# GradientSpaces/LivingScenes

Measured on AMD Instinct MI355X. Metric: object-instances/sec (encode+match+register), N=1024 pts, higher is better.
Workload: dtype f32 (GEMM products as two-piece f16 splits on the f16 matrix cores, fp32 accumulate: as accurate against fp64 as an fp32 FMA chain)

## Files before the change

### livingscenes_amd/csrc/edge.hip

```cpp
#include "ls_launch.h"
#include "ls_device.h"

namespace ls {

constexpr int EK = 16;

__global__ __launch_bounds__(256) void edge_l0_kernel(const float* __restrict__ pts, const int32_t* __restrict__ knn,
                                                      const float* __restrict__ w0, int N, int Co, float oms,
                                                      float* __restrict__ out, int total) {
    const int lane = threadIdx.x & 63, wave = threadIdx.x >> 6;
    const int sub = lane >> 5, o = lane & 31;
    int pid = (xcd_remap(blockIdx.x, gridDim.x) * 4 + wave) * 2 + sub;
    const bool live = pid < total;
    if (!live) pid = total - 1;
    const int b = pid / N;
    const float* P = pts + (size_t)b * N * 3;
    const float cx = pts[(size_t)pid * 3 + 0], cy = pts[(size_t)pid * 3 + 1], cz = pts[(size_t)pid * 3 + 2];
    const float inv = 1.0f / fmaxf(sqrtf(cx * cx + cy * cy + cz * cz), 1e-12f);
    const float ax = cx * inv, ay = cy * inv, az = cz * inv;
    const int32_t* ki = knn + (size_t)pid * EK;
    __shared__ __attribute__((aligned(16))) float l_edge[4][2][EK][8];
    if (o < EK) {
        const int r = ki[o];
        const float nx = P[(size_t)r * 3 + 0], ny = P[(size_t)r * 3 + 1], nz = P[(size_t)r * 3 + 2];
// ... 250 lines not shown
    for (int col = tid; col < 3 * Co; col += 256) {
        const int ax = col / Co, c = col - ax * Co;
        const float* sp = &l_score[ax * 4 + (c & 3)][c >> 2];
        float a = 0.f;
#pragma unroll
        for (int pw = 0; pw < PW; ++pw) a += sp[(pw / PPW) * 64 + (pw % PPW) * LPP];
        cp[col] = a;
    }
}

template <int LPP, int NCH>
__global__ __launch_bounds__(256) void edge_attn_v4_kernel(const float* __restrict__ T, int ldt, const float* __restrict__ Tq, int ldq,
                                                           int NQ, int q_via_rows, const int32_t* __restrict__ knn,
                                                           const int32_t* __restrict__ dst_rows, int Nd, int Ns, int Co,
                                                           float oms, float inv_sqrt_dk, float* __restrict__ out, int total,
                                                           float* __restrict__ rowmax, float* __restrict__ colsum) {
    constexpr int PPW = 64 / LPP;
    __shared__ float l_score[NCH][EK][256];
    __shared__ float l_ssk[EK][256];
    const int tid = threadIdx.x, lane = tid & 63, wave = tid >> 6;
    const int sub = lane / LPP, ll = lane % LPP;
    int pid = (xcd_remap(blockIdx.x, gridDim.x) * 4 + wave) * PPW + sub;
    const bool live = pid < total;
    if (!live) pid = total - 1;
    const int b = pid / Nd;
    const int drow = (dst_rows && q_via_rows) ? dst_rows[pid] : (pid % Nd);
    const float* Tb = T + (size_t)b * Ns * 3 * ldt;
    const float* Td = Tq + ((size_t)b * NQ + drow) * 3 * ldq;
    const int32_t* ki = knn + (size_t)pid * EK;

    F43 qf[NCH];
    float ssq = 0.f;
#pragma unroll
    for (int ch = 0; ch < NCH; ++ch) {
        const int c4 = (ch * LPP + ll) * 4;
        qf[ch] = ld43(Td + 4 * Co + c4, ldq);
        const F43 kd = ld43(Td + 5 * Co + c4, ldq);
        act43(qf[ch], kd, oms);
        ssq += dot43(qf[ch], qf[ch]);
    }
    const float inv_q = inv_fro(group_sum<LPP>(ssq));

#pragma unroll
    for (int ch = 0; ch < NCH; ++ch) {
        const int c4 = (ch * LPP + ll) * 4;
        const F43 ql = ld43(Td + 2 * Co + c4, ldq), qd = ld43(Td + 3 * Co + c4, ldq);
#pragma unroll 2
        for (int k = 0; k < EK; ++k) {
            const float* Tr = Tb + (size_t)ki[k] * 3 * ldt;
            F43 y = add43(ld43(Tr + 2 * Co + c4, ldt), ql);
            const F43 kd = add43(ld43(Tr + 3 * Co + c4, ldt), qd);
            act43(y, kd, oms);
            const float s2 = dot43(y, y);
            l_ssk[k][tid] = (ch == 0) ? s2 : l_ssk[k][tid] + s2;
            l_score[ch][k][tid] = quad_sum(dot43(y, qf[ch]));
        }
    }
    float mx[NCH], sum[NCH];
#pragma unroll
    for (int ch = 0; ch < NCH; ++ch) { mx[ch] = -INFINITY; sum[ch] = 0.f; }
#pragma unroll 4
    for (int k = 0; k < EK; ++k) {
        const float invk = inv_fro(group_sum<LPP>(l_ssk[k][tid]));
#pragma unroll
        for (int ch = 0; ch < NCH; ++ch) {
            const float v = l_score[ch][k][tid] * inv_q * invk * inv_sqrt_dk;
            l_score[ch][k][tid] = v;
            mx[ch] = fmaxf(mx[ch], v);
        }
    }
#pragma unroll
    for (int ch = 0; ch < NCH; ++ch) {
#pragma unroll 4
        for (int k = 0; k < EK; ++k) {
            const float ex = expf(l_score[ch][k][tid] - mx[ch]);
            l_score[ch][k][tid] = ex;
            sum[ch] += ex;
        }
    }

    float rmx = 0.f, rmy = 0.f, rmz = 0.f;
#pragma unroll
    for (int ch = 0; ch < NCH; ++ch) {
        const int c4 = (ch * LPP + ll) * 4;
        const F43 ql = ld43(Td + c4, ldq), qd = ld43(Td + Co + c4, ldq);
        F43 acc;
        acc.x = acc.y = acc.z = make_float4(0.f, 0.f, 0.f, 0.f);
#pragma unroll 2
        for (int k = 0; k < EK; ++k) {
            const float* Tr = Tb + (size_t)ki[k] * 3 * ldt;
            F43 y = add43(ld43(Tr + c4, ldt), ql);
            const F43 kd = add43(ld43(Tr + Co + c4, ldt), qd);
            act43(y, kd, oms);
            const float w = l_score[ch][k][tid];
            fma43(acc, w, y);
        }
        const float inv = 1.0f / sum[ch];
        const float4 ox = make_float4(acc.x.x * inv, acc.x.y * inv, acc.x.z * inv, acc.x.w * inv);
        const float4 oy = make_float4(acc.y.x * inv, acc.y.y * inv, acc.y.z * inv, acc.y.w * inv);
        const float4 oz = make_float4(acc.z.x * inv, acc.z.y * inv, acc.z.z * inv, acc.z.w * inv);
        if (live) {
            float* op = out + (size_t)pid * 3 * Co + c4;
            *reinterpret_cast<float4*>(op) = ox;
            *reinterpret_cast<float4*>(op + Co) = oy;
            *reinterpret_cast<float4*>(op + 2 * Co) = oz;
        }
        rmx = fmaxf(rmx, amax_f4(ox)); rmy = fmaxf(rmy, amax_f4(oy)); rmz = fmaxf(rmz, amax_f4(oz));
        if constexpr (NCH == 1) {
            if (colsum) attn_colsum<LPP>(l_score[0], ox, oy, oz, live, tid, colsum + (size_t)xcd_remap(blockIdx.x, gridDim.x) * 3 * Co);
        }
    }
    if (rowmax) {
        rmx = group_max<LPP>(rmx); rmy = group_max<LPP>(rmy); rmz = group_max<LPP>(rmz);
        if (live && ll == 0) { float* rp = rowmax + (size_t)pid * 3; rp[0] = rmx; rp[1] = rmy; rp[2] = rmz; }
    }
}


__global__ __launch_bounds__(64) void edge_presplit_wq_kernel(const float* __restrict__ W, int rows, int Cin, int KS, uint4* __restrict__ planes,
                                                               float* __restrict__ winv) {
    const int tile = blockIdx.x / KS, ks = blockIdx.x % KS, lane = threadIdx.x;
    const int n = tile * 32 + (lane & 31), k = ks * 16 + 8 * (lane >> 5);
    const float* wr = W + (size_t)min(n, rows - 1) * Cin;
    float am = 0.f;
    for (int c = 0; c < Cin; ++c) am = fmaxf(am, fabsf(wr[c]));
    float sc, inv;
    pow2_scale(am, sc, inv);
    if (ks == 0 && lane < 32 && n < rows) winv[n] = inv;
    __attribute__((aligned(16))) float v[8];
#pragma unroll
    for (int c = 0; c < 8; ++c) v[c] = wr[k + c] * sc;
    f16x8_t h, l;
    split8_f16(v, h, l);
    planes[((size_t)blockIdx.x * 2) * 64 + lane] = __builtin_bit_cast(uint4, h);
    planes[((size_t)blockIdx.x * 2 + 1) * 64 + lane] = __builtin_bit_cast(uint4, l);
}
static size_t edge_wq_plane_count(int Co, int Cin) { return (size_t)(6 * Co / 32) * (Cin / 16) * 2 * 64; }
size_t edge_wq_planes_bytes(int Co, int Cin) { return edge_wq_plane_count(Co, Cin) * sizeof(uint4) + (size_t)6 * Co * sizeof(float); }
int edge_presplit_wq_launch(const float* Wq, int Co, int Cin, void* planes, hipStream_t st) {
    hipLaunchKernelGGL(edge_presplit_wq_kernel, dim3((6 * Co / 32) * (Cin / 16)), dim3(64), 0, st, Wq, 6 * Co, Cin, Cin / 16, (uint4*)planes,
                       (float*)((uint4*)planes + edge_wq_plane_count(Co, Cin)));
    LS_LAUNCH_CHECK();
    return LS_OK;
}

template <int LPP, int CIN>
__global__ __launch_bounds__(256) __attribute__((amdgpu_waves_per_eu(3))) void edge_attn_fq_kernel(const float* __restrict__ T, int ldt, const float* __restrict__ cur,
                                                           const uint4* __restrict__ Wp, const int32_t* __restrict__ knn,
                                                           const int32_t* __restrict__ dst_rows, int Nd, int Ns, float oms, float inv_sqrt_dk,
                                                           float* __restrict__ out, int total, float* __restrict__ rowmax, float* __restrict__ colsum) {
    constexpr int PPW = 64 / LPP, PW = 4 * PPW, ROWS = 3 * PW, MT = (ROWS + 31) / 32, Co = LPP * 4, SC = 2 * Co, NT = SC / 32, SLD = SC + 4,
                  KS = CIN / 16, ASTR = CIN * 2 + 16;
    static_assert(MT * NT == 8, "two output tiles per wave");
    __shared__ float l_score[EK][256];
    __shared__ __attribute__((aligned(16))) float slab[ROWS * SLD];
    __shared__ __attribute__((aligned(16))) char a_pl[2][MT * 32 * ASTR];
    __shared__ int a_inv[MT * 32];
    const float* __restrict__ winv = reinterpret_cast<const float*>(Wp + (size_t)(6 * Co / 32) * KS * 128);
    const int tid = threadIdx.x, lane = tid & 63, wave = tid >> 6;
    const int sub = lane / LPP, ll = lane % LPP;
    const int pid0 = xcd_remap(blockIdx.x, gridDim.x) * PW;
    const int pwl = wave * PPW + sub;
    int pid = pid0 + pwl;
    const bool live = pid < total;
    if (!live) pid = total - 1;
    const int b = pid / Nd;
    const float* Tb = T + (size_t)b * Ns * 3 * ldt;
    const int32_t* ki = knn + (size_t)pid * EK;
    const int c4 = ll * 4;

    uint4 wfh[2][KS], wfl[2][KS];
    auto qload = [&](int cb) {
        const uint4* wt = Wp + (size_t)(cb / 32) * KS * 128 + lane;
#pragma unroll
        for (int u = 0; u < (MT == 2 ? 1 : 2); ++u) {
            const int nt = MT == 2 ? wave : wave + 4 * u;
#pragma unroll
            for (int ks = 0; ks < KS; ++ks) {
                wfh[u][ks] = wt[((size_t)(nt * KS + ks) * 2) * 64];
                wfl[u][ks] = wt[((size_t)(nt * KS + ks) * 2 + 1) * 64];
            }
        }
    };
    qload(4 * Co);
    for (int c = tid; c < MT * 32 * (CIN / 4); c += 256) {
        const int r = c / (CIN / 4), kq = c - r * (CIN / 4);
        uint2 h = make_uint2(0u, 0u), l = make_uint2(0u, 0u);
        float4 v = make_float4(0.f, 0.f, 0.f, 0.f);
        if (r < ROWS) {
            const int pw = r / 3, x = r - 3 * pw;
            const int pa = min(pid0 + pw, total - 1), ba = pa / Nd;
            const int sp = dst_rows ? dst_rows[pa] : pa - ba * Nd;
            v = *reinterpret_cast<const float4*>(cur + (((size_t)ba * Ns + sp) * 3 + x) * CIN + kq * 4);
        }
        {
            float am = fmaxf(fmaxf(fabsf(v.x), fabsf(v.y)), fmaxf(fabsf(v.z), fabsf(v.w)));
            am = max8(am);
            if constexpr (CIN == 64) am = dpp_max<0x140>(am);
            float sc, inv;
            pow2_scale(am, sc, inv);
            if (kq == 0) a_inv[r] = pow2_e(inv);
            split2_f16_pair(f32x2_t{v.x * sc, v.y * sc}, h.x, l.x);
            split2_f16_pair(f32x2_t{v.z * sc, v.w * sc}, h.y, l.y);
        }
        *reinterpret_cast<uint2*>(&a_pl[0][r * ASTR + kq * 8]) = h;
        *reinterpret_cast<uint2*>(&a_pl[1][r * ASTR + kq * 8]) = l;
    }
    __syncthreads();

    auto qmma = [&](int cb) {
        __builtin_amdgcn_sched_barrier(0);
#pragma unroll
        for (int u = 0; u < 2; ++u) {
            const int mt = MT == 2 ? u : 0, nt = MT == 2 ? wave : wave + 4 * u;
            const int aoff = (32 * mt + (lane & 31)) * ASTR + (lane >> 5) * 16;
            f32x16_t acc;
#pragma unroll
            for (int r = 0; r < 16; ++r) acc[r] = 0.f;
#pragma unroll
            for (int ks = 0; ks < KS; ++ks) {
                const f16x8_t ah = __builtin_bit_cast(f16x8_t, *reinterpret_cast<const uint4*>(&a_pl[0][aoff + ks * 32]));
                const f16x8_t al = __builtin_bit_cast(f16x8_t, *reinterpret_cast<const uint4*>(&a_pl[1][aoff + ks * 32]));
                const f16x8_t bh = __builtin_bit_cast(f16x8_t, wfh[MT == 2 ? 0 : u][ks]);
                const f16x8_t bl = __builtin_bit_cast(f16x8_t, wfl[MT == 2 ? 0 : u][ks]);
                acc = __builtin_amdgcn_mfma_f32_32x32x16_f16(al, bh, acc, 0, 0, 0);
                acc = __builtin_amdgcn_mfma_f32_32x32x16_f16(ah, bh, acc, 0, 0, 0);
                acc = __builtin_amdgcn_mfma_f32_32x32x16_f16(ah, bl, acc, 0, 0, 0);
            }
            const int row0 = 32 * mt + 4 * (lane >> 5);
            float* sp = slab + row0 * SLD + 32 * nt + (lane & 31);
            const int ce = pow2_e(winv[cb + 32 * nt + (lane & 31)]);
#pragma unroll
            for (int r = 0; r < 16; ++r) {
                const int dr = (r & 3) + 8 * (r >> 2);
                if (row0 + dr < ROWS) sp[dr * SLD] = scale_pow2(acc[r], a_inv[row0 + dr] + ce);
            }
        }
    };
    const float* srow = slab + 3 * pwl * SLD + c4;
    auto lds43 = [&](int col) {
        F43 r;
        r.x = *reinterpret_cast<const float4*>(srow + col);
        r.y = *reinterpret_cast<const float4*>(srow + SLD + col);
        r.z = *reinterpret_cast<const float4*>(srow + 2 * SLD + col);
        return r;
    };

    qmma(4 * Co);
    __syncthreads();
    qload(2 * Co);
    F43 qf = lds43(0);
    {
        const F43 kd = lds43(Co);
        act43(qf, kd, oms);
    }
    const float inv_q = inv_fro(group_sum<LPP>(dot43(qf, qf)));
    __syncthreads();

    unsigned nb[EK / 2];
    {
        const int4* kp = reinterpret_cast<const int4*>(ki);
#pragma unroll
        for (int u = 0; u < EK / 4; ++u) { const int4 v = kp[u]; nb[2 * u] = (unsigned)v.x | ((unsigned)v.y << 16); nb[2 * u + 1] = (unsigned)v.z | ((unsigned)v.w << 16); }
    }
    const unsigned row_bytes = 3u * (unsigned)ldt * 4u;
    const unsigned lane_off = (unsigned)c4 * 4u;
    const unsigned inst_row = (unsigned)b * (unsigned)Ns;
    auto noff = [&](int k) { return __umul24(inst_row + ((k & 1) ? nb[k >> 1] >> 16 : nb[k >> 1] & 0xFFFFu), row_bytes) + lane_off; };
    auto ldrow = [&](unsigned off, int col) {
        asm volatile("" : "+v"(off));
        F43 r;
        r.x = *reinterpret_cast<const float4*>(reinterpret_cast<const char*>(T + col) + off);
        r.y = *reinterpret_cast<const float4*>(reinterpret_cast<const char*>(T + ldt + col) + off);
        r.z = *reinterpret_cast<const float4*>(reinterpret_cast<const char*>(T + 2 * ldt + col) + off);
        return r;
    };
    qmma(2 * Co);
    __syncthreads();
    {
        constexpr int DP = 2;
        F43 py[DP], pd[DP];
#pragma unroll
        for (int d = 0; d < DP; ++d) { const unsigned o = noff(d); py[d] = ldrow(o, 2 * Co); pd[d] = ldrow(o, 3 * Co); }
        const F43 ql = lds43(0), qd = lds43(Co);
#pragma unroll
        for (int k = 0; k < EK; ++k) {
            F43 y = py[k % DP], kd = pd[k % DP];
            if (k + DP < EK) { const unsigned o = noff(k + DP); py[k % DP] = ldrow(o, 2 * Co); pd[k % DP] = ldrow(o, 3 * Co); }
            __builtin_amdgcn_sched_barrier(0);
            y = add43(y, ql);
            kd = add43(kd, qd);
            act43(y, kd, oms);
            const float invk = inv_fro(group_sum<LPP>(dot43(y, y)));
            l_score[k][tid] = quad_sum(dot43(y, qf)) * inv_q * invk * inv_sqrt_dk;
            __builtin_amdgcn_sched_barrier(0);
        }
    }
#pragma unroll
    for (int k = 0; k < EK / 2; ++k) asm volatile("" : "+v"(nb[k]));
    __syncthreads();
    qload(0);
    float mx = -INFINITY, sum = 0.f;
#pragma unroll 4
    for (int k = 0; k < EK; ++k) mx = fmaxf(mx, l_score[k][tid]);
#pragma unroll 4
    for (int k = 0; k < EK; ++k) {
        const float ex = expf(l_score[k][tid] - mx);
        l_score[k][tid] = ex;
        sum += ex;
    }
    qmma(0);
    __syncthreads();

    {
        const F43 ql = lds43(0), qd = lds43(Co);
        F43 acc;
        acc.x = acc.y = acc.z = make_float4(0.f, 0.f, 0.f, 0.f);
        constexpr int DP = 2;
        F43 py[DP], pd[DP];
#pragma unroll
        for (int d = 0; d < DP; ++d) { const unsigned o = noff(d); py[d] = ldrow(o, 0); pd[d] = ldrow(o, Co); }
#pragma unroll
        for (int k = 0; k < EK; ++k) {
            F43 y = py[k % DP], kd = pd[k % DP];
            if (k + DP < EK) { const unsigned o = noff(k + DP); py[k % DP] = ldrow(o, 0); pd[k % DP] = ldrow(o, Co); }
            __builtin_amdgcn_sched_barrier(0);
            y = add43(y, ql);
            kd = add43(kd, qd);
            act43(y, kd, oms);
            const float w = l_score[k][tid];
            fma43(acc, w, y);
            __builtin_amdgcn_sched_barrier(0);
        }
        const float inv = 1.0f / sum;
        const float4 ox = make_float4(acc.x.x * inv, acc.x.y * inv, acc.x.z * inv, acc.x.w * inv);
        const float4 oy = make_float4(acc.y.x * inv, acc.y.y * inv, acc.y.z * inv, acc.y.w * inv);
        const float4 oz = make_float4(acc.z.x * inv, acc.z.y * inv, acc.z.z * inv, acc.z.w * inv);
        if (live) {
            float* op = out + (size_t)pid * 3 * Co + c4;
            *reinterpret_cast<float4*>(op) = ox;
            *reinterpret_cast<float4*>(op + Co) = oy;
            *reinterpret_cast<float4*>(op + 2 * Co) = oz;
        }
        if (rowmax) {
            const float rmx = group_max<LPP>(amax_f4(ox)), rmy = group_max<LPP>(amax_f4(oy)), rmz = group_max<LPP>(amax_f4(oz));
            if (live && ll == 0) { float* rp = rowmax + (size_t)pid * 3; rp[0] = rmx; rp[1] = rmy; rp[2] = rmz; }
        }
        if (colsum) attn_colsum<LPP>(l_score, ox, oy, oz, live, tid, colsum + (size_t)(pid0 / PW) * 3 * Co);
    }
}

int edge_l0_launch(const float* pts, const int32_t* knn, const float* w0, int B, int N, int Co, float neg_slope, float* out,
                   hipStream_t st) {
    const int total = B * N;
    hipLaunchKernelGGL(edge_l0_kernel, dim3(cdiv(total, 8)), dim3(256), 0, st, pts, knn, w0, N, Co, 1.0f - neg_slope, out, total);
    LS_LAUNCH_CHECK();
    return LS_OK;
}

int edge_run(const Edge& e, const EdgePlan& p, hipStream_t st) {
    if (p.kernel == EdgeKernel::FT_128 || p.kernel == EdgeKernel::FT_256) return edge_ft_attn_launch(e, p, st);
    const float *T = e.T, *Tq = e.T + p.q_off;
    const int total = e.B * e.Nd, Nd = e.Nd, Ns = e.Ns, Co = e.Co;
    const float oms = 1.0f - e.neg_slope, isd = 1.0f / sqrtf(3.0f * e.head_c);
    float* rowmax = p.rowmax_parts ? e.rowmax : nullptr;
    float* colsum = p.cs_rows ? e.colsum : nullptr;
    const dim3 grid(p.grid), block(p.block);
    LS_REQUIRE(p.kernel < EdgeKernel::ATTN || (e.head_c == 16 && Co % 16 == 0 && p.lds <= 64 * 1024),
               "edge_attn: head width must be 16 and divide Co, Co at most 512 (head_c=%d Co=%d)", e.head_c, Co);
#define LS_POOL(K) hipLaunchKernelGGL(K, grid, block, 0, st, T, p.ldp, Tq, p.ldq, p.NQ, p.qvr, e.knn, e.dst_rows, Nd, Ns, oms, e.out, total)
#define LS_V4(LPP, NCH) hipLaunchKernelGGL((edge_attn_v4_kernel<LPP, NCH>), grid, block, 0, st, T, p.ldp, Tq, p.ldq, p.NQ, p.qvr, e.knn, e.dst_rows, Nd, Ns, Co, oms, isd, e.out, total, rowmax, colsum)
#define LS_FQ(LPP, CIN) hipLaunchKernelGGL((edge_attn_fq_kernel<LPP, CIN>), grid, block, 0, st, T, p.ldp, e.cur, (const uint4*)e.planes, e.knn, e.dst_rows, Nd, Ns, oms, isd, e.out, total, rowmax, colsum)
    switch (p.kernel) {
    case EdgeKernel::ATTN_FQ_16_32: LS_FQ(16, 32); break;
    case EdgeKernel::ATTN_FQ_16_64: LS_FQ(16, 64); break;
    case EdgeKernel::ATTN_FQ_32_64: LS_FQ(32, 64); break;
    case EdgeKernel::POOL_V4_8: LS_POOL(edge_pool_v4_kernel<8>); break;
    case EdgeKernel::POOL_V4_16: LS_POOL(edge_pool_v4_kernel<16>); break;
    case EdgeKernel::POOL:
        hipLaunchKernelGGL(edge_pool_kernel, grid, block, 0, st, T, p.ldp, Tq, p.ldq, p.NQ, p.qvr, e.knn, e.dst_rows, Nd, Ns, Co, oms, e.out, total);
        break;
    case EdgeKernel::ATTN_V4_16: LS_V4(16, 1); break;
    case EdgeKernel::ATTN_V4_32: LS_V4(32, 1); break;
    case EdgeKernel::ATTN_V4_64: LS_V4(64, 1); break;
    case EdgeKernel::ATTN_V4_64X2: LS_V4(64, 2); break;
    case EdgeKernel::ATTN:
        hipLaunchKernelGGL(edge_attn_kernel, grid, block, p.lds, st, T, p.ldp, Tq, p.ldq, p.NQ, p.qvr, e.knn, e.dst_rows, Nd, Ns, Co, oms, isd, e.out, total);
        break;
    default: LS_REQUIRE(false, "edge_run: the plan names no kernel of edge.hip");
    }
#undef LS_POOL
#undef LS_V4
#undef LS_FQ
    LS_LAUNCH_CHECK();
    return LS_OK;
}

}
```

### livingscenes_amd/csrc/knn_mfma.hip

```cpp
#include "knn_common.h"
#include "ls_launch.h"

namespace ls {


template <int CC>
struct QuadRow {
    float4 v[6];
    __device__ __forceinline__ void load(const float* __restrict__ row, int lane, int round = 0) {
        const int off = round * 32 + (lane & 3) * 8;
#pragma unroll
        for (int x = 0; x < 3; ++x)
#pragma unroll
            for (int h = 0; h < 2; ++h) v[x * 2 + h] = *reinterpret_cast<const float4*>(row + x * CC + off + 4 * h);
    }
};
template <int CC, bool FMA, bool LAST>
__device__ __forceinline__ float quad_round(float d, const QuadRow<CC>& q, const QuadRow<CC>& c) {
#pragma clang fp contract(off)
    float t[24];
#pragma unroll
    for (int h = 0; h < 2; ++h)
#pragma unroll
        for (int x = 0; x < 3; ++x) {
// ... 9 lines not shown
#pragma unroll
        for (int j = 0; j < 24; ++j) d = FMA ? __builtin_fmaf(t[j], t[j], d) : d + t[j];
        if (s < 3)
            d = __int_as_float(__builtin_amdgcn_update_dpp(0, __float_as_int(d), 0x90, 0xF, 0xF, false));
        else if (!LAST)
            d = __int_as_float(__builtin_amdgcn_update_dpp(0, __float_as_int(d), 0x93, 0xF, 0xF, false));
    }
    return d;
}
template <int CC, bool FMA>
__device__ __forceinline__ float quad_pair_distance(const QuadRow<CC>& q0, const float* __restrict__ qrow, const float* __restrict__ crow,
                                                    int lane) {
    QuadRow<CC> c;
    c.load(crow, lane, 0);
    if constexpr (CC == 32) {
        return quad_round<CC, FMA, true>(0.0f, q0, c);
    } else {
        float d = quad_round<CC, FMA, false>(0.0f, q0, c);
#pragma unroll
        for (int r = 1; r < CC / 32; ++r) {
            QuadRow<CC> q;
            q.load(qrow, lane, r);
            c.load(crow, lane, r);
            d = (r == CC / 32 - 1) ? quad_round<CC, FMA, true>(d, q, c) : quad_round<CC, FMA, false>(d, q, c);
        }
        return d;
    }
}

constexpr int KNN_CENTRE_ROWS = 16;
template <int KK, int WPT>
__global__ __launch_bounds__(64 * WPT) void knn_prep_f16_tile_kernel(const float* __restrict__ f, const float* __restrict__ fc, int Nc, int N, int Npad,
                                                                    unsigned short* __restrict__ out, float* __restrict__ norms, float* __restrict__ iscale,
                                                                    int32_t* __restrict__ zero_buf, long long zero_n) {
    constexpr int D = KK * 16, KPW = KK / WPT, DW = KPW * 16;
    static_assert(KK % WPT == 0 && DW <= 64, "a wave's dims fit one lane each for the centre");
    __shared__ __attribute__((aligned(16))) float lmu[WPT][64];
    __shared__ float lamax[WPT][32], lsum[WPT][32];
    for (long long i = (long long)blockIdx.x * (64 * WPT) + threadIdx.x; i < zero_n; i += (long long)gridDim.x * (64 * WPT)) zero_buf[i] = 0;
    const int lane = threadIdx.x & 63, w = __builtin_amdgcn_readfirstlane(threadIdx.x >> 6), j = lane & 31, h = lane >> 5;
    const int tpi = Npad >> 5, b = blockIdx.x / tpi, tile = blockIdx.x % tpi, r = tile * 32 + j;
    const bool live = r < N;
    const float* rp = f + ((size_t)b * N + (live ? r : 0)) * D + w * DW + h * 8;
    float4 x[KPW][2];
#pragma unroll
    for (int kk = 0; kk < KPW; ++kk) { x[kk][0] = *reinterpret_cast<const float4*>(rp + kk * 16); x[kk][1] = *reinterpret_cast<const float4*>(rp + kk * 16 + 4); }
    {
        const int nc = min(Nc, KNN_CENTRE_ROWS);
        const float* cp = fc + (size_t)b * Nc * D + w * DW + lane;
        if (lane < DW) {
            float v[KNN_CENTRE_ROWS];
#pragma unroll
            for (int rr = 0; rr < KNN_CENTRE_ROWS; ++rr) v[rr] = cp[(size_t)min(rr, max(nc - 1, 0)) * D];
            float s0 = 0.f, s1 = 0.f, s2 = 0.f, s3 = 0.f;
#pragma unroll
            for (int rr = 0; rr < KNN_CENTRE_ROWS; rr += 4) {
                if (rr + 3 < nc) { s0 += v[rr]; s1 += v[rr + 1]; s2 += v[rr + 2]; s3 += v[rr + 3]; }
                else {
#pragma unroll
                    for (int u = 0; u < 3; ++u) if (rr + u < nc) s0 += v[rr + u];
                }
            }
            lmu[w][lane] = ((s0 + s1) + (s2 + s3)) / (float)nc;
        }
        __builtin_amdgcn_s_waitcnt(0xc07f);
        __builtin_amdgcn_wave_barrier();
    }
    float c[KPW][8];
    float amax = 0.f;
#pragma unroll
    for (int kk = 0; kk < KPW; ++kk) {
        const float4 m0 = *reinterpret_cast<const float4*>(&lmu[w][kk * 16 + h * 8]), m1 = *reinterpret_cast<const float4*>(&lmu[w][kk * 16 + h * 8 + 4]);
        const float4 x0 = x[kk][0], x1 = x[kk][1];
        const float t[8] = {x0.x - m0.x, x0.y - m0.y, x0.z - m0.z, x0.w - m0.w, x1.x - m1.x, x1.y - m1.y, x1.z - m1.z, x1.w - m1.w};
#pragma unroll
        for (int i = 0; i < 8; ++i) { c[kk][i] = live ? t[i] : 0.f; amax = fmaxf(amax, fabsf(t[i])); }
    }
    amax = fmaxf(amax, __shfl_xor(amax, 32, 64));
    if (h == 0) lamax[w][j] = amax;
    __syncthreads();
#pragma unroll
    for (int u = 0; u < WPT; ++u) amax = fmaxf(amax, lamax[u][j]);
    float sc;
    const unsigned be = pow2_scale_be(amax, sc);
    sc = live ? sc : 0.f;
    unsigned short* op = out + ((((size_t)b * tpi + tile) * KK + w * KPW) * 64 + lane) * 8;
    float s = 0.f;
#pragma unroll
    for (int kk = 0; kk < KPW; ++kk) {
        unsigned pk[4];
#pragma unroll
        for (int i = 0; i < 4; ++i) {
            const float c0 = c[kk][2 * i], c1 = c[kk][2 * i + 1];
            s += c0 * c0 + c1 * c1;
            const f16x2_t hv = __builtin_convertvector(f32x2_t{c0 * sc, c1 * sc}, f16x2_t);
            pk[i] = __builtin_bit_cast(unsigned, hv);
        }
        uint4 wv;
        wv.x = pk[0]; wv.y = pk[1]; wv.z = pk[2]; wv.w = pk[3];
        *reinterpret_cast<uint4*>(op + (size_t)kk * 512) = wv;
    }
    s += __shfl_xor(s, 32, 64);
    if (h == 0) lsum[w][j] = s;
    __syncthreads();
    if (w == 0 && h == 0 && live) {
        float t = lsum[0][j];
#pragma unroll
        for (int u = 1; u < WPT; ++u) t += lsum[u][j];
        norms[(size_t)b * N + r] = t;
        iscale[(size_t)b * N + r] = pow2_inv(be);
    }
}
#ifndef LS_KF_PK
#define LS_KF_PK 1
#endif
constexpr int KF_LCAP = 64;

template <int CC>
struct KfLds {
    float qrows[KF_QT][3 * CC];
    float qnx[KF_QT], qny[KF_QT];
    unsigned hm[KF_QT][64];
    float T[KF_QT];
    int cnt[KF_QT];
    int base[KF_QT + 1];
    unsigned short list[KF_QT][KF_LCAP];
    unsigned plist[KF_QT * KF_LCAP];
    u64 keys[KF_QT][KF_LCAP];
};

template <int CC, bool FMA>
__device__ __noinline__ u64 kf_brute_row(const float* __restrict__ qrow, const float* __restrict__ sbase, int Ns, int lane) {
    constexpr int RF = 3 * CC;
    const int quad = lane >> 2;
    const bool qlast = (lane & 3) == 3;
    QuadRow<CC> qv;
    qv.load(qrow, lane);
    u64 best = ~0ull;
    for (int base = 0; base < Ns; base += 48) {
        u64 ks[3];
#pragma unroll
        for (int u = 0; u < 3; ++u) {
            const int c = base + u * 16 + quad;
            const bool v = c < Ns;
            ks[u] = make_key(quad_pair_distance<CC, FMA>(qv, qrow, sbase + (size_t)(v ? c : 0) * RF, lane), c, v & qlast);
        }
        const int src = ((lane & 15) << 2) + 3;
        const u64 n0 = bperm64(src, ks[0]), n1 = bperm64(src, ks[1]), n2 = bperm64(src, ks[2]);
        u64 k = lane < 16 ? best : (lane < 32 ? n0 : (lane < 48 ? n1 : n2));
        LS_SORT64(cx64, k, lane)
        best = k;
    }
    return best;
}

template <int CC, bool FMA, int TPW>
__global__ __launch_bounds__(64 * KF_WAVES, FMA ? 3 : 4) void knn_fused_kernel(const float* __restrict__ dstf, const float* __restrict__ srcf, const int32_t* __restrict__ dst_rows,
                                                                  const unsigned short* __restrict__ dq, const unsigned short* __restrict__ sq,
                                                                  const float* __restrict__ nrm_dst, const float* __restrict__ nrm_src,
                                                                  const float* __restrict__ isc_dst, const float* __restrict__ isc_src, int Nd, int dst_n,
                                                                  int dst_npad, int Ns, int ns_pad, int K, int qtiles, float eps,
                                                                  int32_t* __restrict__ idx_out, float* __restrict__ dist_out, int32_t* __restrict__ surv_cnt) {
    constexpr int D = 3 * CC, KK = D / 16, RF = 3 * CC;
    __shared__ __attribute__((aligned(16))) KfLds<CC> L;
    const int tid = threadIdx.x, lane = tid & 63;
    const int wave = __builtin_amdgcn_readfirstlane(tid >> 6);
    const int l31 = lane & 31, lh = lane >> 5;
    const int logical = xcd_remap(blockIdx.x, gridDim.x);
    const int b = logical / qtiles, q0 = (logical - b * qtiles) * KF_QT;
    const unsigned short* dqb = dq + (size_t)b * dst_npad * D;
    const unsigned short* sqb = sq + (size_t)b * ns_pad * D;
    const float* sbase = srcf + (size_t)b * Ns * RF;
    const float* dbase = dstf + (size_t)b * dst_n * RF;
    const int ntiles = ns_pad >> 5;

    for (int i = tid; i < KF_QT * (RF / 4); i += 64 * KF_WAVES) {
        const int qr = i / (RF / 4), c4 = i - qr * (RF / 4);
        const int q = min(q0 + qr, Nd - 1);
        const int r = dst_rows ? dst_rows[(size_t)b * Nd + q] : q;
        *reinterpret_cast<float4*>(&L.qrows[qr][c4 * 4]) = *reinterpret_cast<const float4*>(dbase + (size_t)r * RF + c4 * 4);
    }
    if (tid < KF_QT) {
        const int q = q0 + tid;
        const int r = q < Nd ? (dst_rows ? dst_rows[(size_t)b * Nd + q] : q) : 0;
        const float nq = nrm_dst[(size_t)b * dst_n + r], iq = isc_dst[(size_t)b * dst_n + r];
        L.qnx[tid] = q < Nd ? nq : 0.f;
        L.qny[tid] = q < Nd ? -2.0f * iq : 0.f;
        L.cnt[tid] = 0;
    }
    for (int i = tid; i < KF_QT * 64; i += 64 * KF_WAVES) (&L.hm[0][0])[i] = 0x7F800000u;

    f16x8_t a[KK];
    {
        const int qi = q0 + l31;
        const int r = qi < Nd ? (dst_rows ? dst_rows[(size_t)b * Nd + qi] : qi) : 0;
        const unsigned short* ap = dqb + ((size_t)(r >> 5) * KK * 64 + lh * 32 + (r & 31)) * 8;
#pragma unroll
        for (int kk = 0; kk < KK; ++kk) a[kk] = __builtin_bit_cast(f16x8_t, *reinterpret_cast<const uint4*>(ap + (size_t)kk * 512));
    }
    f32x16_t S[TPW];
    float cns[TPW], cic[TPW];
    {
        f16x8_t bf[2][KK];
        auto load_b = [&](int t, f16x8_t (&dstb)[KK]) {
            const int tg = min(wave + KF_WAVES * t, ntiles - 1);
            const unsigned short* bp = sqb + ((size_t)tg * KK * 64 + lane) * 8;
#pragma unroll
            for (int kk = 0; kk < KK; ++kk) dstb[kk] = __builtin_bit_cast(f16x8_t, *reinterpret_cast<const uint4*>(bp + (size_t)kk * 512));
        };
        load_b(0, bf[0]);
#pragma unroll
        for (int t = 0; t < TPW; ++t) {
            if (t + 1 < TPW) load_b(t + 1, bf[(t + 1) & 1]);
            const int cg = min((wave + KF_WAVES * t) * 32 + l31, Ns - 1);
            cns[t] = nrm_src[(size_t)b * Ns + cg];
            cic[t] = isc_src[(size_t)b * Ns + cg];
#pragma unroll
            for (int r = 0; r < 16; ++r) S[t][r] = 0.0f;
#pragma unroll
            for (int kk = 0; kk < KK; ++kk) S[t] = __builtin_amdgcn_mfma_f32_32x32x16_f16(a[kk], bf[t & 1][kk], S[t], 0, 0, 0);
        }
    }
    __syncthreads();
    bool colv[TPW];
#pragma unroll
    for (int t = 0; t < TPW; ++t) colv[t] = (wave + KF_WAVES * t) < ntiles && (wave + KF_WAVES * t) * 32 + l31 < Ns;
#if LS_KF_PK
    {
        const int slot = (wave & 1) * 32 + l31;
        f32x2_t cn2[TPW], ci2[TPW];
#pragma unroll
        for (int t = 0; t < TPW; ++t) { const float cn = colv[t] ? cns[t] : INFINITY; cn2[t] = f32x2_t{cn, cn}; ci2[t] = f32x2_t{cic[t], cic[t]}; }
        const f32x2_t eps2 = {eps, eps};
#pragma unroll
        for (int r = 0; r < 16; r += 2) {
            const int qr = (r & 3) + 8 * (r >> 2) + 4 * lh;
            const f32x2_t qx = *reinterpret_cast<const f32x2_t*>(&L.qnx[qr]), qy = *reinterpret_cast<const f32x2_t*>(&L.qny[qr]);
            float hm0 = INFINITY, hm1 = INFINITY;
#pragma unroll
            for (int t = 0; t < TPW; ++t) {
                const f32x2_t nn = qx + cn2[t], w = qy * ci2[t];
                const f32x2_t sv = {S[t][r], S[t][r + 1]};
                const f32x2_t dh = __builtin_elementwise_fma(sv, w, nn), e = eps2 * nn;
                const f32x2_t hi = dh + e;
                f32x2_t lo = dh - e;
                hm0 = fminf(hm0, hi.x); hm1 = fminf(hm1, hi.y);
                asm volatile("" : "+v"(lo));
                S[t][r] = lo.x; S[t][r + 1] = lo.y;
            }
            const float h0 = fmaxf(hm0, 0.0f), h1 = fmaxf(hm1, 0.0f);
            if (h0 < INFINITY) atomicMin(&L.hm[qr][slot], __float_as_uint(h0));
            if (h1 < INFINITY) atomicMin(&L.hm[qr + 1][slot], __float_as_uint(h1));
            if ((r & 3) == 2) __builtin_amdgcn_sched_barrier(0);
        }
    }
#else
    {
        const int slot = (wave & 1) * 32 + l31;
#pragma unroll
        for (int r = 0; r < 16; ++r) {
            const int qr = (r & 3) + 8 * (r >> 2) + 4 * lh;
            const float2 qn = make_float2(L.qnx[qr], L.qny[qr]);
            float hmin = INFINITY;
#pragma unroll
            for (int t = 0; t < TPW; ++t) {
                const float nn = qn.x + cns[t], w = qn.y * cic[t];
                const float dh = __builtin_fmaf(S[t][r], w, nn), e = eps * nn;
                hmin = colv[t] ? fminf(hmin, dh + e) : hmin;
                float lo = dh - e;
                asm volatile("" : "+v"(lo));
                S[t][r] = lo;
            }
            const float h = fmaxf(hmin, 0.0f);
            if (h < INFINITY) atomicMin(&L.hm[qr][slot], __float_as_uint(h));
            if ((r & 3) == 3) __builtin_amdgcn_sched_barrier(0);
        }
    }
#endif
    __syncthreads();
#pragma unroll
    for (int u = 0; u < KF_QT / KF_WAVES; ++u) {
        const int qr = wave * (KF_QT / KF_WAVES) + u;
        const unsigned tb = kth_smallest_upper_bound(L.hm[qr][lane], K < 64 ? K : 64);
        if (lane == 0) L.T[qr] = __uint_as_float(tb);
    }
    __syncthreads();
    {
        unsigned mask[TPW];
#pragma unroll
        for (int t = 0; t < TPW; ++t) mask[t] = 0;
#pragma unroll
        for (int r = 0; r < 16; ++r) {
            const float Tr = L.T[(r & 3) + 8 * (r >> 2) + 4 * lh];
#pragma unroll
            for (int t = 0; t < TPW; ++t) mask[t] |= (S[t][r] > Tr) ? 0u : (1u << r);
        }
#pragma unroll
        for (int t = 0; t < TPW; ++t) {
            const int cg = (wave + KF_WAVES * t) * 32 + l31;
            unsigned m = colv[t] ? mask[t] : 0u;
            while (m) {
                const int r = __builtin_ctz(m);
                m &= m - 1;
                const int qr = (r & 3) + 8 * (r >> 2) + 4 * lh;
                if (q0 + qr < Nd) {
                    const int pos = atomicAdd(&L.cnt[qr], 1);
                    if (pos < KF_LCAP) L.list[qr][pos] = (unsigned short)cg;
                }
            }
        }
    }
    __syncthreads();
    if (wave == 0) {
        const int c = (lane < KF_QT && L.cnt[lane] <= KF_LCAP) ? L.cnt[lane] : 0;
        int incl = c;
#pragma unroll
        for (int o = 1; o < KF_QT; o <<= 1) {
            const int v = __shfl_up(incl, o, 64);
            incl += lane >= o ? v : 0;
        }
        if (lane < KF_QT) L.base[lane] = incl - c;
        if (lane == KF_QT - 1) L.base[KF_QT] = incl;
        if (lane < KF_QT && q0 + lane < Nd && surv_cnt) surv_cnt[(size_t)b * Nd + q0 + lane] = -(L.cnt[lane] > KF_LCAP ? Ns : L.cnt[lane]) - 1;
    }
    __syncthreads();
    for (int i = tid; i < KF_QT * KF_LCAP; i += 64 * KF_WAVES) {
        const int qr = i / KF_LCAP, j = i - qr * KF_LCAP;
        const int c = L.cnt[qr];
        if (c <= KF_LCAP && j < c) L.plist[L.base[qr] + j] = (unsigned)L.list[qr][j] | ((unsigned)qr << 16) | ((unsigned)j << 21);
    }
    __syncthreads();
    {
        const int P = L.base[KF_QT];
        const int Q = wave * 16 + (lane >> 2);
        const bool qlast = (lane & 3) == 3;
        struct Pair { unsigned ent; bool v; QuadRow<CC> c; };
        auto fetch = [&](int p0, Pair& pr) {
            const int p = p0 + Q;
            pr.v = p < P;
            pr.ent = L.plist[pr.v ? p : 0];
            pr.c.load(sbase + (size_t)(pr.ent & 0xFFFFu) * RF, lane, 0);
        };
        auto finish = [&](const Pair& pr) {
            const int cand = pr.ent & 0xFFFFu, qr = (pr.ent >> 16) & 31, slot = pr.ent >> 21;
            const float* qrow = &L.qrows[qr][0];
            QuadRow<CC> qv;
            qv.load(qrow, lane);
            float d;
            if constexpr (CC == 32) {
                d = quad_round<CC, FMA, true>(0.0f, qv, pr.c);
            } else {
                const float* crow = sbase + (size_t)cand * RF;
                d = quad_round<CC, FMA, false>(0.0f, qv, pr.c);
#pragma unroll
                for (int r = 1; r < CC / 32; ++r) {
                    QuadRow<CC> q, c;
                    q.load(qrow, lane, r);
                    c.load(crow, lane, r);
                    d = (r == CC / 32 - 1) ? quad_round<CC, FMA, true>(d, q, c) : quad_round<CC, FMA, false>(d, q, c);
                }
            }
            if (pr.v && qlast) L.keys[qr][slot] = make_key(d, cand, true);
        };
// ... 106 lines not shown
```

Before: 57940.

## Prefetch gathers and staging loads ahead of MFMA phases in edge-attn and knn

In the edge attention kernel, the staging loads of cur rows, the knn indices, the per-column scale values and the first neighbour-row gathers are issued into registers before the preceding MFMA phase or barrier. This lets their global-memory latency overlap with matrix-core work. In the knn kernel, query rows and norms are loaded into registers with one dst_rows lookup per lane broadcast by shuffle, and the LDS stores are placed before or after the first B-tile load depending on the template configuration. The cost is higher register pressure, which may reduce occupancy.

```diff
diff --git a/livingscenes_amd/csrc/edge.hip b/livingscenes_amd/csrc/edge.hip
--- a/livingscenes_amd/csrc/edge.hip
+++ b/livingscenes_amd/csrc/edge.hip
@@ -426,6 +426,11 @@
     constexpr int PPW = 64 / LPP, PW = 4 * PPW, ROWS = 3 * PW, MT = (ROWS + 31) / 32, Co = LPP * 4, SC = 2 * Co, NT = SC / 32, SLD = SC + 4,
                   KS = CIN / 16, ASTR = CIN * 2 + 16;
     static_assert(MT * NT == 8, "two output tiles per wave");
+#ifndef LS_FQ_GB
+#define LS_FQ_GB (LPP == 16)
+#define LS_FQ_GC (LPP == 16)
+#endif
+    constexpr bool FQ_GB = LS_FQ_GB, FQ_GC = LS_FQ_GC;
     __shared__ float l_score[EK][256];
     __shared__ __attribute__((aligned(16))) float slab[ROWS * SLD];
     __shared__ __attribute__((aligned(16))) char a_pl[2][MT * 32 * ASTR];
@@ -444,6 +449,7 @@
     const int c4 = ll * 4;
 
     uint4 wfh[2][KS], wfl[2][KS];
+    float wiv[2];
     auto qload = [&](int cb) {
         const uint4* wt = Wp + (size_t)(cb / 32) * KS * 128 + lane;
 #pragma unroll
@@ -454,19 +460,49 @@
                 wfh[u][ks] = wt[((size_t)(nt * KS + ks) * 2) * 64];
                 wfl[u][ks] = wt[((size_t)(nt * KS + ks) * 2 + 1) * 64];
             }
+            wiv[u] = winv[cb + 32 * nt + (lane & 31)];
         }
     };
+    constexpr int ST = MT * 32 * (CIN / 4) / 256;
+    static_assert(ST * 256 == MT * 32 * (CIN / 4), "whole staging trips");
+    int s_pa[ST], s_sp[ST];
+#pragma unroll
+    for (int t = 0; t < ST; ++t) {
+        const int r = min((tid + 256 * t) / (CIN / 4), ROWS - 1);
+        s_pa[t] = min(pid0 + r / 3, total - 1);
+    }
+    if (dst_rows) {
+#pragma unroll
+        for (int t = 0; t < ST; ++t) s_sp[t] = dst_rows[s_pa[t]];
+    } else {
+#pragma unroll
+        for (int t = 0; t < ST; ++t) s_sp[t] = s_pa[t] - (s_pa[t] / Nd) * Nd;
+    }
+    int4 kiv[EK / 4];
+#pragma unroll
+    for (int u = 0; u < EK / 4; ++u) kiv[u] = reinterpret_cast<const int4*>(ki)[u];
     qload(4 * Co);
-    for (int c = tid; c < MT * 32 * (CIN / 4); c += 256) {
+    float4 s_v[ST];
+#pragma unroll
+    for (int t = 0; t < ST; ++t) {
+        const int c = tid + 256 * t;
+        const int r = min(c / (CIN / 4), ROWS - 1), kq = c % (CIN / 4);
+        const int x = r - 3 * (r / 3);
+        const int ba = s_pa[t] / Nd;
+        if ((256 * t) / (CIN / 4) < ROWS)
+            s_v[t] = *reinterpret_cast<const float4*>(cur + (((size_t)ba * Ns + s_sp[t]) * 3 + x) * CIN + kq * 4);
+        else
+            s_v[t] = make_float4(0.f, 0.f, 0.f, 0.f);
+    }
+    __builtin_amdgcn_sched_barrier(0);
+#pragma unroll
+    for (int t = 0; t < ST; ++t) asm volatile("" : "+v"(s_v[t].x), "+v"(s_v[t].y), "+v"(s_v[t].z), "+v"(s_v[t].w));
+#pragma unroll
+    for (int t = 0; t < ST; ++t) {
+        const int c = tid + 256 * t;
         const int r = c / (CIN / 4), kq = c - r * (CIN / 4);
         uint2 h = make_uint2(0u, 0u), l = make_uint2(0u, 0u);
-        float4 v = make_float4(0.f, 0.f, 0.f, 0.f);
-        if (r < ROWS) {
-            const int pw = r / 3, x = r - 3 * pw;
-            const int pa = min(pid0 + pw, total - 1), ba = pa / Nd;
-            const int sp = dst_rows ? dst_rows[pa] : pa - ba * Nd;
-            v = *reinterpret_cast<const float4*>(cur + (((size_t)ba * Ns + sp) * 3 + x) * CIN + kq * 4);
-        }
+        const float4 v = r < ROWS ? s_v[t] : make_float4(0.f, 0.f, 0.f, 0.f);
         {
             float am = fmaxf(fmaxf(fabsf(v.x), fabsf(v.y)), fmaxf(fabsf(v.z), fabsf(v.w)));
             am = max8(am);
@@ -480,9 +516,12 @@
         *reinterpret_cast<uint2*>(&a_pl[0][r * ASTR + kq * 8]) = h;
         *reinterpret_cast<uint2*>(&a_pl[1][r * ASTR + kq * 8]) = l;
     }
-    __syncthreads();
-
-    auto qmma = [&](int cb) {
+    unsigned nb[EK / 2];
+#pragma unroll
+    for (int u = 0; u < EK / 4; ++u) { const int4 v = kiv[u]; nb[2 * u] = (unsigned)v.x | ((unsigned)v.y << 16); nb[2 * u + 1] = (unsigned)v.z | ((unsigned)v.w << 16); }
+    __syncthreads();
+
+    auto qmma = [&]() {
         __builtin_amdgcn_sched_barrier(0);
 #pragma unroll
         for (int u = 0; u < 2; ++u) {
@@ -503,7 +542,7 @@
             }
             const int row0 = 32 * mt + 4 * (lane >> 5);
             float* sp = slab + row0 * SLD + 32 * nt + (lane & 31);
-            const int ce = pow2_e(winv[cb + 32 * nt + (lane & 31)]);
+            const int ce = pow2_e(wiv[MT == 2 ? 0 : u]);
 #pragma unroll
             for (int r = 0; r < 16; ++r) {
                 const int dr = (r & 3) + 8 * (r >> 2);
@@ -520,7 +559,7 @@
         return r;
     };
 
-    qmma(4 * Co);
+    qmma();
     __syncthreads();
     qload(2 * Co);
     F43 qf = lds43(0);
@@ -531,12 +570,6 @@
     const float inv_q = inv_fro(group_sum<LPP>(dot43(qf, qf)));
     __syncthreads();
 
-    unsigned nb[EK / 2];
-    {
-        const int4* kp = reinterpret_cast<const int4*>(ki);
-#pragma unroll
-        for (int u = 0; u < EK / 4; ++u) { const int4 v = kp[u]; nb[2 * u] = (unsigned)v.x | ((unsigned)v.y << 16); nb[2 * u + 1] = (unsigned)v.z | ((unsigned)v.w << 16); }
-    }
     const unsigned row_bytes = 3u * (unsigned)ldt * 4u;
     const unsigned lane_off = (unsigned)c4 * 4u;
     const unsigned inst_row = (unsigned)b * (unsigned)Ns;
@@ -549,13 +582,17 @@
         r.z = *reinterpret_cast<const float4*>(reinterpret_cast<const char*>(T + 2 * ldt + col) + off);
         return r;
     };
-    qmma(2 * Co);
+    constexpr int DP = 2;
+    F43 py[DP], pd[DP];
+    auto gfirst = [&](int cy, int cd) {
+#pragma unroll
+        for (int d = 0; d < DP; ++d) { const unsigned o = noff(d); py[d] = ldrow(o, cy); pd[d] = ldrow(o, cd); }
+    };
+    if constexpr (FQ_GB) gfirst(2 * Co, 3 * Co);
+    qmma();
     __syncthreads();
     {
-        constexpr int DP = 2;
-        F43 py[DP], pd[DP];
-#pragma unroll
-        for (int d = 0; d < DP; ++d) { const unsigned o = noff(d); py[d] = ldrow(o, 2 * Co); pd[d] = ldrow(o, 3 * Co); }
+        if constexpr (!FQ_GB) gfirst(2 * Co, 3 * Co);
         const F43 ql = lds43(0), qd = lds43(Co);
 #pragma unroll
         for (int k = 0; k < EK; ++k) {
@@ -583,17 +620,15 @@
         l_score[k][tid] = ex;
         sum += ex;
     }
-    qmma(0);
+    if constexpr (FQ_GC) gfirst(0, Co);
+    qmma();
     __syncthreads();
 
     {
         const F43 ql = lds43(0), qd = lds43(Co);
         F43 acc;
         acc.x = acc.y = acc.z = make_float4(0.f, 0.f, 0.f, 0.f);
-        constexpr int DP = 2;
-        F43 py[DP], pd[DP];
-#pragma unroll
-        for (int d = 0; d < DP; ++d) { const unsigned o = noff(d); py[d] = ldrow(o, 0); pd[d] = ldrow(o, Co); }
+        if constexpr (!FQ_GC) gfirst(0, Co);
 #pragma unroll
         for (int k = 0; k < EK; ++k) {
             F43 y = py[k % DP], kd = pd[k % DP];
diff --git a/livingscenes_amd/csrc/knn_mfma.hip b/livingscenes_amd/csrc/knn_mfma.hip
--- a/livingscenes_amd/csrc/knn_mfma.hip
+++ b/livingscenes_amd/csrc/knn_mfma.hip
@@ -185,6 +185,21 @@
         best = k;
     }
     return best;
+}
+
+template <int CC, int QTRIPS>
+__device__ __forceinline__ void kf_put_queries(KfLds<CC>& L, const float4 (&qv)[QTRIPS], float qnx, float qny, int tid, int l31) {
+    constexpr int RF = 3 * CC;
+#pragma unroll
+    for (int t = 0; t < QTRIPS; ++t) {
+        const int i = min(tid + 64 * KF_WAVES * t, KF_QT * (RF / 4) - 1);
+        const int qr = i / (RF / 4), c4 = i - qr * (RF / 4);
+        *reinterpret_cast<float4*>(&L.qrows[qr][c4 * 4]) = qv[t];
+    }
+    L.qnx[l31] = qnx;
+    L.qny[l31] = qny;
+    L.cnt[l31] = 0;
+    for (int i = tid; i < KF_QT * 64; i += 64 * KF_WAVES) (&L.hm[0][0])[i] = 0x7F800000u;
 }
 
 template <int CC, bool FMA, int TPW>
@@ -207,27 +222,24 @@
     const float* dbase = dstf + (size_t)b * dst_n * RF;
     const int ntiles = ns_pad >> 5;
 
-    for (int i = tid; i < KF_QT * (RF / 4); i += 64 * KF_WAVES) {
+    const int qi = q0 + l31;
+    const int rq = dst_rows ? dst_rows[(size_t)b * Nd + min(qi, Nd - 1)] : min(qi, Nd - 1);
+    const int ra = qi < Nd ? rq : 0;
+    constexpr int QTRIPS = (KF_QT * (RF / 4) + 64 * KF_WAVES - 1) / (64 * KF_WAVES);
+    float4 qv[QTRIPS];
+#pragma unroll
+    for (int t = 0; t < QTRIPS; ++t) {
+        const int i = min(tid + 64 * KF_WAVES * t, KF_QT * (RF / 4) - 1);
         const int qr = i / (RF / 4), c4 = i - qr * (RF / 4);
-        const int q = min(q0 + qr, Nd - 1);
-        const int r = dst_rows ? dst_rows[(size_t)b * Nd + q] : q;
-        *reinterpret_cast<float4*>(&L.qrows[qr][c4 * 4]) = *reinterpret_cast<const float4*>(dbase + (size_t)r * RF + c4 * 4);
-    }
-    if (tid < KF_QT) {
-        const int q = q0 + tid;
-        const int r = q < Nd ? (dst_rows ? dst_rows[(size_t)b * Nd + q] : q) : 0;
-        const float nq = nrm_dst[(size_t)b * dst_n + r], iq = isc_dst[(size_t)b * dst_n + r];
-        L.qnx[tid] = q < Nd ? nq : 0.f;
-        L.qny[tid] = q < Nd ? -2.0f * iq : 0.f;
-        L.cnt[tid] = 0;
-    }
-    for (int i = tid; i < KF_QT * 64; i += 64 * KF_WAVES) (&L.hm[0][0])[i] = 0x7F800000u;
-
+        const int r = __shfl(rq, qr);
+        qv[t] = *reinterpret_cast<const float4*>(dbase + (size_t)r * RF + c4 * 4);
+    }
+    const float nq = nrm_dst[(size_t)b * dst_n + ra], iq = isc_dst[(size_t)b * dst_n + ra];
+    constexpr bool Q_FIRST = CC == 64 && TPW == 4;
+    if constexpr (Q_FIRST) kf_put_queries<CC, QTRIPS>(L, qv, qi < Nd ? nq : 0.f, qi < Nd ? -2.0f * iq : 0.f, tid, l31);
     f16x8_t a[KK];
     {
-        const int qi = q0 + l31;
-        const int r = qi < Nd ? (dst_rows ? dst_rows[(size_t)b * Nd + qi] : qi) : 0;
-        const unsigned short* ap = dqb + ((size_t)(r >> 5) * KK * 64 + lh * 32 + (r & 31)) * 8;
+        const unsigned short* ap = dqb + ((size_t)(ra >> 5) * KK * 64 + lh * 32 + (ra & 31)) * 8;
 #pragma unroll
         for (int kk = 0; kk < KK; ++kk) a[kk] = __builtin_bit_cast(f16x8_t, *reinterpret_cast<const uint4*>(ap + (size_t)kk * 512));
     }
@@ -242,6 +254,7 @@
             for (int kk = 0; kk < KK; ++kk) dstb[kk] = __builtin_bit_cast(f16x8_t, *reinterpret_cast<const uint4*>(bp + (size_t)kk * 512));
         };
         load_b(0, bf[0]);
+        if constexpr (!Q_FIRST) kf_put_queries<CC, QTRIPS>(L, qv, qi < Nd ? nq : 0.f, qi < Nd ? -2.0f * iq : 0.f, tid, l31);
 #pragma unroll
         for (int t = 0; t < TPW; ++t) {
             if (t + 1 < TPW) load_b(t + 1, bf[(t + 1) & 1]);
```

After: 58140 (median of 5 runs). About the same (+0.3%).
